# Nemo1999/Joint-TensoRF

Hardware: AMD Instinct MI355X
Metric: train rays/sec & Msamples/sec composited, lego VM-48, 1/2/4/8 MI355X (higher is better)
Workload: dtype f32; 1 GPU; bat_blender_VM stage 4: grid 400x400x400, S=1000 samples/ray, 1955 rays/iter/GPU (all_view_rand_grid lattice over 100 views), blur off, full train step (fwd+loss+bwd+Adam+pose Adam); samples_per_ray=1000, launch=eager, parallelism=1 GPU

## Files before the change

### joint_tensorf_amd/csrc/jt_shade.hip

```cpp
#include <atomic>
#include <cstdlib>

#include "jt_common.h"
#include "jt_walk.h"

#include "jt_shade_core.h"

#ifndef JT_B16_PINGPONG
#define JT_B16_PINGPONG 1
#endif
#ifndef JT_BF16X3_DEFAULT
#define JT_BF16X3_DEFAULT 7
#endif

namespace jt {

template <class C, int REC>
__global__ __launch_bounds__(256, 2) void k_shade_fwd(Dev D, MlpDev M, PeMask pm, const float* __restrict__ rays_o,
                                                      const float* __restrict__ rays_d,
                                                      const float* __restrict__ jitter,
                                                      const float* __restrict__ zvals,
                                                      const float* __restrict__ tmin,
                                                      const int* __restrict__ offset, int R,
                                                      const int* __restrict__ eray, const int* __restrict__ esmp,
                                                      const float* __restrict__ vdir, float* __restrict__ rgb_s,
                                                      float* __restrict__ rec, int cap, int rrows) {
  typedef BwdCfg<C> B;
  extern __shared__ __align__(16) float smem[];
  const int total = min(offset[R], cap);
  const int ntiles = (total + 31) >> 5;
  const int nblk = min((int)gridDim.x, (ntiles + 3) / 4);
  if ((int)blockIdx.x >= nblk) return;
  load_weights_lds<C>(smem, M);
  __syncthreads();
  const int lane = threadIdx.x & 63, wv = __builtin_amdgcn_readfirstlane(threadIdx.x >> 6);
  const int j_ = lane & 31, h_ = lane >> 5;
  constexpr int HOFF = (C::KIND == JT_MLP_FEA) ? 0 : 12;
  const XcdShare xs = xcd_share(ntiles, nblk);
  for (int tile = xs.lo + xs.rank * 4 + wv; tile < xs.hi; tile += xs.peers * 4) {
    int j = j_, h = h_;
    asm volatile("" : "+v"(j), "+v"(h));
    const int e = tile * 32 + j;
    const bool on = e < total;
    const int ee = on ? e : total - 1;
    float* rt = REC ? rec + (size_t)tile * (size_t)rrows * 32 : nullptr;
    EntryGeom g = entry_geom(D, rays_o, rays_d, jitter, zvals, tmin, eray, esmp, ee);
    float vd[3] = {vdir[(size_t)ee * 3], vdir[(size_t)ee * 3 + 1], vdir[(size_t)ee * 3 + 2]};
    if (REC && on && h == 0) {
#pragma unroll
      for (int c = 0; c < 3; ++c) {
        if (REC & 1) rec_st(rec_at(rt, B::R_VD + c, 4u * (unsigned)j), vd[c]);
        rec_st(rec_at(rt, B::R_GEO + c, 4u * (unsigned)j), g.n[c]);
      }
    }
    f32x16 facc = gather_basis<C, REC == 1>(D, smem, g.n, j, h, rt, on);
    if (REC) rec_store<1>(rt, B::R_F, &facc, j, h, on);
    Hidden<C> h1 = layer1<C>(smem, facc, vd, pm, j, h);
    relu_<C>(h1);
    if (REC) {
      unsigned mask1 = 0u;
#pragma unroll
      for (int mt = 0; mt < C::MT; ++mt)
#pragma unroll
        for (int r = 0; r < 16; ++r) mask1 |= (h1.v[mt][r] > 0.f) ? (1u << (mt * 16 + r)) : 0u;
      if (on) rec_st(rec_at(rt, B::R_MASK, 4u * (unsigned)j + 128u * (unsigned)h), __uint_as_float(mask1));
      if (REC & 1) rec_store<C::MT>(rt, B::R_H1, h1.v, j, h, on);
    }
    Hidden<C> h2 = layer2<C>(smem, h1, j, h);
    relu_<C>(h2);
    if (REC) {
      unsigned mask2 = 0u;
#pragma unroll
      for (int mt = 0; mt < C::MT; ++mt)
#pragma unroll
        for (int r = 0; r < 16; ++r) mask2 |= (h2.v[mt][r] > 0.f) ? (1u << (mt * 16 + r)) : 0u;
      if (on) rec_st(rec_at(rt, B::R_MASK + 2, 4u * (unsigned)j + 128u * (unsigned)h), __uint_as_float(mask2));
      if (REC & 1) rec_store<C::MT>(rt, B::R_MID + HOFF, h2.v, j, h, on);
      if ((REC & 1) && C::KIND != JT_MLP_FEA) {
        float pe[12];
        view_pe(vd, pm, pe);
        if (on && h == 0) {
#pragma unroll
          for (int k = 0; k < 12; ++k) rec_st(rec_at(rt, B::R_MID + k, 4u * (unsigned)j), pe[k]);
        }
      }
    }
    float o[3];
    layer3<C>(smem, h2, vd, pm, h, o);
    if (on && h == 0) {
#pragma unroll
      for (int c = 0; c < 3; ++c) rgb_s[(size_t)e * 3 + c] = 1.f / (1.f + expf(-o[c]));
    }
  }
}


#if JT_STAMP
__device__ unsigned long long g_stamps[8];
#define JT_STAMP_T() (__builtin_readcyclecounter())
#endif

template <class C, int REC>
__global__ __launch_bounds__(JT_B16_THREADS) void k_shade_fwd_b16(Dev D, MlpDev M, PeMask pm, const float* __restrict__ rays_o,
                                                      const float* __restrict__ rays_d,
                                                      const float* __restrict__ jitter,
                                                      const float* __restrict__ zvals,
                                                      const float* __restrict__ tmin,
                                                      const int* __restrict__ offset, int R,
                                                      const int* __restrict__ eray, const int* __restrict__ esmp,
                                                      const float* __restrict__ vdir, float* __restrict__ rgb_s,
                                                      float* __restrict__ rec, int cap, int rrows) {
  typedef BwdCfg<C> B;
  extern __shared__ __align__(16) unsigned char smem_raw[];
  typedef B16Cfg<C> Q;
  const uint4* img = reinterpret_cast<const uint4*>(smem_raw);
  const float* tail = reinterpret_cast<const float*>(smem_raw + (size_t)Q::V_END * 16);
  const float* smem = tail - C::O_W3;
  const int total = min(offset[R], cap);
  const int ntiles = (total + 31) >> 5;
  constexpr int NW = JT_B16_THREADS / 64;
  const int nblk = min((int)gridDim.x, (ntiles + NW - 1) / NW);
  if ((int)blockIdx.x >= nblk) return;
  load_weights_lds_b16<C>(smem_raw, M);
  __syncthreads();
  const int lane = threadIdx.x & 63, wv = __builtin_amdgcn_readfirstlane(threadIdx.x >> 6);
  const int j_ = lane & 31, h_ = lane >> 5;
  constexpr int HOFF = (C::KIND == JT_MLP_FEA) ? 0 : 12;
  const XcdShare xs = xcd_share(ntiles, nblk);
#if JT_SETPRIO
  if (wv >= NW / 2) __builtin_amdgcn_s_setprio(1);
#endif
  const int stride = xs.peers * NW;
  const int first = xs.lo + xs.rank * NW;
  const int iters0 = first < xs.hi ? (xs.hi - first + stride - 1) / stride : 0;
  f32x16 facc;
  float vd0 = 0.f, vd1 = 0.f, vd2 = 0.f;
  int e = 0;
  bool on = false, have = false;
  float* rt = nullptr;
#pragma unroll
  for (int r = 0; r < 16; ++r) facc[r] = 0.f;
#define JT_FWD_GATHER_STEP \
  {                                                                                                                    \
    int j = j_, h = h_; \
    asm volatile("" : "+v"(j), "+v"(h)); \
    e = tile * 32 + j; \
    on = e < total; \
    const int ee = on ? e : total - 1; \
    rt = REC ? rec + (size_t)tile * (size_t)rrows * 32 : nullptr; \
    EntryGeom g = entry_geom(D, rays_o, rays_d, jitter, zvals, tmin, eray, esmp, ee); \
    vd0 = vdir[(size_t)ee * 3], vd1 = vdir[(size_t)ee * 3 + 1], vd2 = vdir[(size_t)ee * 3 + 2]; \
    const float vd[3] = {vd0, vd1, vd2}; \
    if (REC && on && h == 0) { \
_Pragma("unroll") \
// ... 1098 lines not shown
  __shared__ float s_red[4][16][64];
  const int lane = threadIdx.x & 63, wv = threadIdx.x >> 6;
  const int m = lane & 31, h = lane >> 5;
  const int total = min(offset[R], cap);
  const int n = min(total - chunk_start, chunk_cap);
  if (n <= 0) return;
  const int ntiles = (n + 31) >> 5;
  const int per = wgrad_tiles_per_wave(n, gridDim.x);
  if ((int)blockIdx.x >= wgrad_active_blocks(n, gridDim.x)) return;
  const int w = blockIdx.x * 4 + wv;
  const int t_begin = min(w * per, ntiles), t_end = min(t_begin + per, ntiles);
  f32x16 acc[MT][NT];
  float asum[MT];
#pragma unroll
  for (int a = 0; a < MT; ++a) {
    asum[a] = 0.f;
#pragma unroll
    for (int b = 0; b < NT; ++b)
#pragma unroll
      for (int r = 0; r < 16; ++r) acc[a][b][r] = 0.f;
  }
  const size_t tstride = (size_t)rec_rows * 32;
  auto loadA = [&](int t, float (*dst)[16]) {
#pragma unroll
    for (int a = 0; a < MT; ++a) {
      const int c = a * 32 + m;
      load_row_half(rec + (size_t)t * tstride + (size_t)(a_row0 + min(c, M - 1)) * 32, c < M, h, dst[a]);
    }
  };
  auto prepA = [&](float (*av)[16], int nl, B3 (*a3)[2]) {
#pragma unroll
    for (int a = 0; a < MT; ++a) {
      if (nl < 32) mask_tail(av[a], h, nl);
#pragma unroll
      for (int q = 0; q < 16; ++q) asum[a] += av[a][q];
      a3[a][0] = split8(av[a]);
      a3[a][1] = split8(av[a] + 8);
    }
  };
  float av[MT][16], an[MT][16];
  B3 a3[MT][2];
  float gw[MT][3], raw[XA ? 4 : 1][16], rawn[XA ? 4 : 1][16];
  if (XA) {
#pragma unroll
    for (int a = 0; a < MT; ++a)
#pragma unroll
      for (int c = 0; c < 3; ++c) gw[a][c] = (a * 32 + m < M) ? gs.w3[c * gs.in3 + gs.hoff + a * 32 + m] : 0.f;
  }
  if (XF == 0) {
    auto loadB = [&](int t, int b, float* dst) {
      const int c = b * 32 + m;
      load_row_half(rec + (size_t)t * tstride + (size_t)(b_row0 + min(c, N - 1)) * 32, c < N, h, dst);
    };
    float bv[16], bn[16];
    if (t_begin < t_end) {
      if (XA) g2_load_raw(rec + (size_t)t_begin * tstride, gs, m, h, raw);
      else loadA(t_begin, av);
      loadB(t_begin, 0, bv);
    }
    for (int t = t_begin; t < t_end; ++t) {
      const int nl = min(32, n - t * 32);
#pragma unroll
      for (int b = 0; b < NT; ++b) {
        if (b + 1 < NT) {
          loadB(t, b + 1, bn);
        } else {
          const int tn = min(t + 1, t_end - 1);
          if (XA) g2_load_raw(rec + (size_t)tn * tstride, gs, m, h, rawn);
          else loadA(tn, an);
          loadB(tn, 0, bn);
        }
        if (b == 0) {
          if (XA) {
#pragma unroll
            for (int c = 0; c < 4; ++c) pin16(raw[XA ? c : 0]);
            g2_derive<MT>(raw, gw, m, av);
          } else {
#pragma unroll
          for (int a = 0; a < MT; ++a) pin16(av[a]);
          }
          prepA(av, nl, a3);
        }
        pin16(bv);
        if (nl < 32) mask_tail(bv, h, nl);
        const B3 b0 = split8(bv), b1 = split8(bv + 8);
#pragma unroll
        for (int a = 0; a < MT; ++a) {
          acc[a][b] = mfma6(a3[a][0], b0, acc[a][b]);
          acc[a][b] = mfma6(a3[a][1], b1, acc[a][b]);
        }
#pragma unroll
        for (int q = 0; q < 16; ++q) bv[q] = bn[q];
      }
      if (XA) {
#pragma unroll
        for (int c = 0; c < 4; ++c)
#pragma unroll
          for (int q = 0; q < 16; ++q) raw[XA ? c : 0][q] = rawn[XA ? c : 0][q];
      } else {
#pragma unroll
      for (int a = 0; a < MT; ++a)
#pragma unroll
        for (int q = 0; q < 16; ++q) av[a][q] = an[a][q];
      }
    }
  } else {
    const bool feat = m < APP, view = (XF == 1) && !feat && (m < APP + 3);
    const int srow = feat ? f_row0 + m : vd_row0 + (view ? m - APP : 0);
    const float m0 = view ? pm.v0 : pm.f0, m1 = view ? pm.v1 : pm.f1;
    const bool live = feat || view;
    float x[16], xn[16];
    if (t_begin < t_end) {
      loadA(t_begin, av);
      load_row_half(rec + (size_t)t_begin * tstride + (size_t)srow * 32, live, h, x);
    }
    for (int t = t_begin; t < t_end; ++t) {
      const int nl = min(32, n - t * 32);
      {
        const int tn = min(t + 1, t_end - 1);
        loadA(tn, an);
        load_row_half(rec + (size_t)tn * tstride + (size_t)srow * 32, live, h, xn);
      }
      pin16(x);
#pragma unroll
      for (int a = 0; a < MT; ++a) pin16(av[a]);
      if (nl < 32) mask_tail(x, h, nl);
      prepA(av, nl, a3);
      float sn[16], cs[16];
#pragma unroll
      for (int q = 0; q < 16; ++q) sincos_grad(x[q], &sn[q], &cs[q]);
#pragma unroll
      for (int b = 0; b < NT; ++b) {
        float bv[16];
#pragma unroll
        for (int q = 0; q < 16; ++q) bv[q] = live ? pe_pick<XF>(b, x[q], sn[q], cs[q], m0, m1) : 0.f;
        const B3 b0 = split8(bv), b1 = split8(bv + 8);
#pragma unroll
        for (int a = 0; a < MT; ++a) {
          acc[a][b] = mfma6(a3[a][0], b0, acc[a][b]);
          acc[a][b] = mfma6(a3[a][1], b1, acc[a][b]);
        }
      }
#pragma unroll
      for (int q = 0; q < 16; ++q) x[q] = xn[q];
#pragma unroll
      for (int a = 0; a < MT; ++a)
#pragma unroll
        for (int q = 0; q < 16; ++q) av[a][q] = an[a][q];
    }
  }
  wgrad_epilogue<MT, NT>(acc, asum, s_red, slab, lane, wv, m, h);
}

template <int MT, int NT, int XF>
__device__ inline void wgrad_reduce_body(int xblock, const float* __restrict__ slabs, int blocks_per_chunk,
                                         size_t chunk_stride, int chunk_entries, int total, int M, int N, int APP,
                                         float* __restrict__ dW, int ldw, float* __restrict__ db) {
  const int nchunks = (total + chunk_entries - 1) / chunk_entries;
  constexpr int PER = MT * NT * 1024 + MT * 32;
  const int idx = xblock * blockDim.x + threadIdx.x;
  if (idx >= PER) return;
  float s0 = 0.f, s1 = 0.f, s2 = 0.f, s3 = 0.f;
  const int gy = gridDim.y;
  for (int c = 0; c < nchunks; ++c) {
    const int active = wgrad_active_blocks(min(total - c * chunk_entries, chunk_entries), blocks_per_chunk);
    const float* base = slabs + (size_t)c * chunk_stride + idx;
    int q = blockIdx.y;
    for (; q + 3 * gy < active; q += 4 * gy) {
      s0 += base[(size_t)q * PER];
      s1 += base[(size_t)(q + gy) * PER];
      s2 += base[(size_t)(q + 2 * gy) * PER];
      s3 += base[(size_t)(q + 3 * gy) * PER];
    }
    for (; q < active; q += gy) s0 += base[(size_t)q * PER];
  }
  const float sum = (s0 + s1) + (s2 + s3);
  if (sum == 0.f) return;
  if (idx < MT * NT * 1024) {
    const int tile = idx >> 10, r = (idx >> 6) & 15, lane = idx & 63;
    const int a = tile / NT, b = tile - a * NT, m = lane & 31, h = lane >> 5;
    const int i = a * 32 + rowmap(r, 0) + 4 * h;
    const int k = (XF == 0) ? b * 32 + m : l1_column<XF>(b, m, APP);
    if (i < M && k >= 0 && k < N) atomicAdd(dW + (size_t)i * ldw + k, sum);
  } else if (db) {
    const int i = idx - MT * NT * 1024;
    if (i < M) atomicAdd(db + i, sum);
  }
}

template <class C>
struct WgradDims {
  static constexpr int NT3 = (C::IN3 + 31) / 32, NT1 = 5, NTB = (C::NC + 31) / 32;
  static constexpr size_t P3 = 1 * NT3 * 1024 + 32, P2 = (size_t)C::MT * C::MT * 1024 + C::MT * 32,
                          P1 = (size_t)C::MT * NT1 * 1024 + C::MT * 32, PB = 1 * NTB * 1024 + 32;
};

struct MlpGrad {
  float *basis, *w1, *b1, *w2, *b2, *w3, *b3;
};

template <class C>
__global__ __launch_bounds__(256) void k_wgrad_reduce4(const float* __restrict__ slabs, int blocks_per_chunk,
                                                       size_t chunk_stride, int chunk_entries,
                                                       const int* __restrict__ offset, int R, int cap, MlpGrad GM) {
  typedef WgradDims<C> W;
  constexpr int NT3 = W::NT3, NT1 = W::NT1, NTB = W::NTB;
  constexpr int XF1 = (C::KIND == JT_MLP_FEA) ? 1 : 2;
  constexpr int B3 = (int)((W::P3 + 255) / 256), B2 = (int)((W::P2 + 255) / 256), B1 = (int)((W::P1 + 255) / 256);
  const int total = min(offset[R], cap);
  const float* s3 = slabs;
  const float* s2 = s3 + W::P3 * blocks_per_chunk;
  const float* s1 = s2 + W::P2 * blocks_per_chunk;
  const float* sb = s1 + W::P1 * blocks_per_chunk;
  const int x = blockIdx.x;
  if (x < B3)
    wgrad_reduce_body<1, NT3, 0>(x, s3, blocks_per_chunk, chunk_stride, chunk_entries, total, 3, C::IN3, C::APP,
                                 GM.w3, C::IN3, GM.b3);
  else if (x < B3 + B2)
    wgrad_reduce_body<C::MT, C::MT, 0>(x - B3, s2, blocks_per_chunk, chunk_stride, chunk_entries, total, C::HID, C::HID,
                                       C::APP, GM.w2, C::HID, GM.b2);
  else if (x < B3 + B2 + B1)
    wgrad_reduce_body<C::MT, NT1, XF1>(x - B3 - B2, s1, blocks_per_chunk, chunk_stride, chunk_entries, total, C::HID,
                                       C::IN1, C::APP, GM.w1, C::IN1, GM.b1);
  else
    wgrad_reduce_body<1, NTB, 0>(x - B3 - B2 - B1, sb, blocks_per_chunk, chunk_stride, chunk_entries, total, C::APP, C::NC,
                                 C::APP, GM.basis, C::NC, (float*)nullptr);
}

}

using namespace jt;

static std::atomic<int> g_matrix_mode{-1};
static int bf16x3_mode() {
  int m = g_matrix_mode.load(std::memory_order_relaxed);
  if (m < 0) {
    const char* e = getenv("JT_BF16X3");
    m = (e ? atoi(e) : JT_BF16X3_DEFAULT) & 7;
    g_matrix_mode.store(m, std::memory_order_relaxed);
  }
  return m;
}

typedef ShadeCfg<48, 27, 64, JT_MLP_FEA> CfgBlender;
typedef ShadeCfg<20, 20, 32, JT_MLP_WEAKVIEW> CfgLlff;

static int shade_kind(const JtScene* s) {
  if (!s) return -1;
  if (s->view_pe != 2 || s->fea_pe != 2) return -1;
  if (s->n_comp_app == 48 && s->app_dim == 27 && s->mlp_hidden == 64 && s->mlp_kind == JT_MLP_FEA) return 0;
  if (s->n_comp_app == 20 && s->app_dim == 20 && s->mlp_hidden == 32 && s->mlp_kind == JT_MLP_WEAKVIEW) return 1;
  return -1;
}

static int g_chunk_log2 = 0;
static int chunk_entries() {
  if (!g_chunk_log2) {
    const char* e = getenv("JT_SHADE_CHUNK_LOG2");
    int l = e ? atoi(e) : 22;
    if (l < 16 || l > 22) l = 22;
    g_chunk_log2 = l;
  }
  return 1 << g_chunk_log2;
}
#if JT_STAMP
extern "C" int jt_debug_read_stamps(unsigned long long* out8) {
  if (hipMemcpyFromSymbol(out8, HIP_SYMBOL(g_stamps), 8 * sizeof(unsigned long long)) != hipSuccess) return JT_ERR_ARG;
  unsigned long long z[8] = {0, 0, 0, 0, 0, 0, 0, 0};
  if (hipMemcpyToSymbol(HIP_SYMBOL(g_stamps), z, sizeof(z)) != hipSuccess) return JT_ERR_ARG;
  return JT_OK;
}
#endif
static std::atomic<int> g_bwd_split{-2};
static int scatter_wgs(bool gemms_beside, bool lean = false, bool w12 = false) {
  static const int v = [] { const char* e = getenv("JT_SCATTER_WGS"); const int n = e ? atoi(e) : 0; return n > 0 ? n : 0; }();
  return v ? std::min(v, chip().cus) : chip().wgs(gemms_beside ? ((lean && !w12) ? 224 : 192) : 256);
}
static int bwd_split_mode() {
  int m = g_bwd_split.load(std::memory_order_relaxed);
  if (m < -1) {
    const char* e = getenv("JT_BWD_SPLIT");
    m = e ? atoi(e) : -1;
    if (m != 0 && m != 1 && m != 8 && m != 16) m = -1;
    g_bwd_split.store(m, std::memory_order_relaxed);
  }
  return m;
}
#if JT_TILE_STAMP
extern "C" int jt_debug_read_tile_stamps(unsigned long long* out16) {
  if (hipMemcpyFromSymbol(out16, HIP_SYMBOL(g_tstamps), 16 * sizeof(unsigned long long)) != hipSuccess) return JT_ERR_ARG;
  unsigned long long z[16] = {};
  if (hipMemcpyToSymbol(HIP_SYMBOL(g_tstamps), z, sizeof(z)) != hipSuccess) return JT_ERR_ARG;
  return JT_OK;
}
#endif
static std::atomic<int> g_lean{-1};
static int lean_mode() {
  int m = g_lean.load(std::memory_order_relaxed);
  if (m < 0) {
    const char* e = getenv("JT_LEAN_TAPE");
    m = (e ? atoi(e) : 1) ? 1 : 0;
    g_lean.store(m, std::memory_order_relaxed);
  }
  return m;
}
template <class C>
// ... 83 lines not shown
                             3 * (size_t)kTileMaxTiles * sizeof(int), 3 * (size_t)kTileMaxTiles * sizeof(int),
                             3 * (size_t)kTileMaxTiles * sizeof(int), 64 * sizeof(int)};
    for (int i = 0; i < 7; ++i) out[9 + 2 * i] = (int64_t)(uintptr_t)ptrs[i], out[10 + 2 * i] = (int64_t)sizes[i];
  }
}
extern "C" int jt_shade_workspace_layout(const JtScene* scene, int n_entries_max, int64_t* out23) {
  const int kind = shade_kind(scene);
  if (kind < 0 || !out23) return JT_ERR_UNSUPPORTED;
  if (n_entries_max < 1 || n_entries_max > kMaxEntries) return JT_ERR_ARG;
  if (kind == 0) ws_layout<CfgBlender>(n_entries_max, out23);
  else ws_layout<CfgLlff>(n_entries_max, out23);
  return JT_OK;
}

extern "C" int jt_shade_record_layout(const JtScene* scene, int32_t* out) {
  const int kind = shade_kind(scene);
  if (kind < 0 || !out) return JT_ERR_UNSUPPORTED;
  if (kind == 0) {
    out[0] = rec_rows<CfgBlender>(); out[1] = BwdCfg<CfgBlender>::R_MASK; out[2] = CfgBlender::HID;
  } else {
    out[0] = rec_rows<CfgLlff>(); out[1] = BwdCfg<CfgLlff>::R_MASK; out[2] = CfgLlff::HID;
  }
  out[3] = 32;
  return JT_OK;
}

template <class C, int REC>
static int launch_shade_fwd_t(const Dev& D, const MlpDev& M, const PeMask& pm, const float* rays_o,
                              const float* rays_d, const float* jitter, const float* zvals, const float* tmin,
                              const int32_t* offset, int R, const int32_t* eray, const int32_t* esmp,
                              const float* vdir, float* rgb_s, float* rec, int cap, hipStream_t st) {
  long tiles = ((long)cap + 31) / 32;
  if (bf16x3_mode() & 1) {
    const size_t lds16 = B16Cfg<C>::LDS_BYTES;
    (void)hipFuncSetAttribute(reinterpret_cast<const void*>(k_shade_fwd_b16<C, REC>),
                              hipFuncAttributeMaxDynamicSharedMemorySize, (int)lds16);
    constexpr int NW = JT_B16_THREADS / 64;
    int blocks16 = (int)std::min<long>((tiles + NW - 1) / NW, chip().cus);
    hipLaunchKernelGGL((k_shade_fwd_b16<C, REC>), dim3(blocks16), dim3(JT_B16_THREADS), lds16, st, D, M, pm, rays_o, rays_d, jitter,
                       zvals, tmin, offset, R, eray, esmp, vdir, rgb_s, rec, cap, rec_rows<C>());
    JT_LAUNCH_CHECK();
    return JT_OK;
  }
  const size_t lds = C::LDS_FLOATS * sizeof(float);
  (void)hipFuncSetAttribute(reinterpret_cast<const void*>(k_shade_fwd<C, REC>),
                            hipFuncAttributeMaxDynamicSharedMemorySize, (int)lds);
  int blocks = (int)std::min<long>((tiles + 3) / 4, 512);
  hipLaunchKernelGGL((k_shade_fwd<C, REC>), dim3(blocks), dim3(256), lds, st, D, M, pm, rays_o, rays_d, jitter, zvals,
                     tmin, offset, R, eray, esmp, vdir, rgb_s, rec, cap, rec_rows<C>());
  JT_LAUNCH_CHECK();
  return JT_OK;
}

template <class C>
static int launch_shade_fwd(const Dev& D, const MlpDev& M, const PeMask& pm, const float* rays_o,
                            const float* rays_d, const float* jitter, const float* zvals, const float* tmin,
                            const int32_t* offset, int R, const int32_t* eray, const int32_t* esmp,
                            const float* vdir, float* rgb_s, int cap, float* ws, size_t ws_bytes, int flags,
                            hipStream_t st) {
  if (ws) {
    if (ws_bytes < WsLayout<C>::bytes(cap)) return JT_ERR_ARG;
    if (flags & JT_SHADE_POSE_ONLY)
      return launch_shade_fwd_t<C, 2>(D, M, pm, rays_o, rays_d, jitter, zvals, tmin, offset, R, eray, esmp, vdir,
                                      rgb_s, ws, cap, st);
    if (lean_tape<C>())
      return launch_shade_fwd_t<C, 3>(D, M, pm, rays_o, rays_d, jitter, zvals, tmin, offset, R, eray, esmp, vdir,
                                      rgb_s, ws, cap, st);
    return launch_shade_fwd_t<C, 1>(D, M, pm, rays_o, rays_d, jitter, zvals, tmin, offset, R, eray, esmp, vdir,
                                    rgb_s, ws, cap, st);
  }
  return launch_shade_fwd_t<C, 0>(D, M, pm, rays_o, rays_d, jitter, zvals, tmin, offset, R, eray, esmp, vdir,
                                  rgb_s, nullptr, cap, st);
}

extern "C" int jt_shade_forward(const JtScene* scene, const JtFactors* factors, const JtMlp* mlp, const float* rays_o,
                                const float* rays_d, const float* jitter, const float* zvals, const float* tmin,
                                const int32_t* shade_offset, int n_rays, const int32_t* entry_ray,
                                const int32_t* entry_smp, const float* viewdirs, float* rgb_s, int n_entries_max,
                                void* workspace, size_t workspace_bytes, int flags, void* stream) {
  Dev D;
  int rc = make_dev(scene, factors, &D);
  if (rc) return rc;
  if (!factors || !mlp || !rays_o || !rays_d || !tmin || !shade_offset || !entry_ray || !entry_smp || !viewdirs ||
      !rgb_s)
    return JT_ERR_ARG;
  if (!mlp->basis || !mlp->w1 || !mlp->b1 || !mlp->w2 || !mlp->b2 || !mlp->w3 || !mlp->b3) return JT_ERR_ARG;
  if (D.ndc && !zvals) return JT_ERR_ARG;
  const int kind = shade_kind(scene);
  if (kind < 0) return JT_ERR_UNSUPPORTED;
  if (n_entries_max < 1) return JT_OK;
  if (n_entries_max > kMaxEntries) return JT_ERR_ARG;
  MlpDev M = {mlp->basis, mlp->w1, mlp->b1, mlp->w2, mlp->b2, mlp->w3, mlp->b3};
  PeMask pm = pe_masks(scene->fea_pe_progress, scene->view_pe_progress, scene->fea_pe, scene->view_pe);
  hipStream_t st = (hipStream_t)stream;
  if (kind == 0)
    return launch_shade_fwd<CfgBlender>(D, M, pm, rays_o, rays_d, jitter, zvals, tmin, shade_offset, n_rays,
                                        entry_ray, entry_smp, viewdirs, rgb_s, n_entries_max, (float*)workspace,
                                        workspace_bytes, flags, st);
  return launch_shade_fwd<CfgLlff>(D, M, pm, rays_o, rays_d, jitter, zvals, tmin, shade_offset, n_rays, entry_ray,
                                   entry_smp, viewdirs, rgb_s, n_entries_max, (float*)workspace, workspace_bytes, flags,
                                   st);
}

template <class C>
struct TileSel {
  static constexpr int NG = (C::CA + 15) / 16;
  static constexpr int SPLIT0 = (NG >= 3) ? 2 : 0;
  static int ch_max(int cfg) { return (cfg == 0 && SPLIT0) ? 16 * SPLIT0 : C::CA; }
  static int waves(int cfg) { return cfg == 0 ? 16 : 8; }
  static size_t lds_bytes(int cfg, int line_len) { return tile_lds_bytes(line_len, ch_max(cfg), waves(cfg)); }
  static int tiles(int H, int W) { return tiles_along(W) * tiles_along(H); }
  template <int CFG>
  static int launch(const Dev& D, const MlpDev& M, const JtFactors& G, const TileWs& TW, const int32_t* offset, int R,
                    float* g_xyz, const float* rc, int start, int ccap, int cap, int line_len, hipStream_t st) {
    constexpr int SPLIT = CFG == 0 ? SPLIT0 : 0;
    constexpr int WAVES = CFG == 0 ? 16 : 8;
    constexpr int NCLS = SPLIT ? 2 : 1;
    int nt[3], ntmax = 1;
    for (int a = 0; a < 3; ++a) nt[a] = tiles(D.ph[a], D.pw[a]), ntmax = std::max(ntmax, nt[a]);
    const int nblk = (ccap + 255) / 256;
    hipLaunchKernelGGL(k_tile_zero, dim3((ntmax + 255) / 256, 3), dim3(256), 0, st, TW, nt[0], nt[1], nt[2]);
    hipLaunchKernelGGL((k_tile_bin<C, false>), dim3(nblk), dim3(256), 0, st, D, TW, offset, R, rc, start, ccap, cap);
    hipLaunchKernelGGL(k_tile_scan, dim3(3), dim3(1024), 0, st, TW, nt[0], nt[1], nt[2]);
    hipLaunchKernelGGL((k_tile_bin<C, true>), dim3(nblk), dim3(256), 0, st, D, TW, offset, R, rc, start, ccap, cap);
    const size_t lds = lds_bytes(CFG, line_len);
    static size_t attr = 0;
    if (attr < lds) {
      if (hipFuncSetAttribute(reinterpret_cast<const void*>(k_tile_scatter<C, SPLIT, WAVES>),
                              hipFuncAttributeMaxDynamicSharedMemorySize, (int)lds) != hipSuccess)
        return JT_ERR_UNSUPPORTED;
      attr = lds;
    }
    static const int nwg_env = [] { const char* e = getenv("JT_TILE_WGS"); const int v = e ? atoi(e) : 0; return v >= 6 ? v : 0; }();
    const int nwg = nwg_env ? nwg_env : std::max(chip().cus, 6);
    static const int ratio = [] { const char* e = getenv("JT_TILE_RATIO"); const int v = e ? atoi(e) : 0; return (v > 0 && v < 100) ? v : 62; }();
    TileClasses TC;
    int acc = 0;
    for (int pl = 0; pl < 3; ++pl) {
      const int share = nwg / 3 + (pl < nwg % 3 ? 1 : 0);
      const int c0 = NCLS == 2 ? std::max(1, std::min(share - 1, share * ratio / 100)) : share;
      TC.start[pl * NCLS] = acc;
      acc += c0;
      if (NCLS == 2) {
        TC.start[pl * NCLS + 1] = acc;
        acc += share - c0;
      }
    }
    for (int k = 3 * NCLS; k <= kTileMaxClasses; ++k) TC.start[k] = acc;
    hipLaunchKernelGGL((k_tile_scatter<C, SPLIT, WAVES>), dim3(acc), dim3(WAVES * 64), lds, st, D, M, G, TW, rc, TC);
    hipLaunchKernelGGL(k_tile_gxyz, dim3(nblk), dim3(256), 0, st, TW, 3 * NCLS, offset, R, g_xyz, start, ccap, cap);
    return JT_OK;
  }
};

template <class C>
static int launch_shade_bwd(const Dev& D, const MlpDev& M, const PeMask& pm, const JtFactors& G, const JtMlp& GM,
                            const int32_t* offset, int R, const float* rgb_s, const float* g_rgb_s, float* g_xyz,
                            int cap,
                            float* ws, size_t ws_bytes, int flags, hipStream_t st, hipStream_t aux,
                            hipEvent_t ev_fork, hipEvent_t ev_join) {
  typedef BwdCfg<C> B;
  typedef WsLayout<C> W;
  const size_t lds = B::LDS_FLOATS * sizeof(float);
  if (lds > 160 * 1024) return JT_ERR_UNSUPPORTED;
  if (ws_bytes < W::bytes(cap)) return JT_ERR_ARG;
  const int chunk = kChunkEntries;
  const int nchunks = (int)(((long)cap + chunk - 1) / chunk);
  (void)hipFuncSetAttribute(reinterpret_cast<const void*>(k_shade_bwd<C, false>),
                            hipFuncAttributeMaxDynamicSharedMemorySize, (int)lds);
  (void)hipFuncSetAttribute(reinterpret_cast<const void*>(k_shade_bwd<C, true>),
                            hipFuncAttributeMaxDynamicSharedMemorySize, (int)lds);
  float* recs = ws;
  float* slabs = ws + W::rec_floats(cap);
  const size_t cstride = W::slab_floats_per_chunk();
  const int nb = kWgradBlocks;
  static const int abl_env = [] { const char* e = getenv("JT_ABLATE"); return e ? atoi(e) : 0; }();
  const int det = jt_deterministic();
  const int ablate = abl_env | ((flags & JT_SHADE_SKIP_WGRAD) ? 4 : 0) |
                     ((flags & kNoGradRecords) ? 2 : 0) | (det ? 16 : 0) | (lean_tape<C>() ? 32 : 0);
  constexpr int NT3 = W::NT3, NT1 = W::NT1, NTB = W::NTB;
  constexpr int XF1 = (C::KIND == JT_MLP_FEA) ? 1 : 2;
  const bool use_aux = aux && ev_fork && ev_join && !(ablate & 4);
  static const bool pipe = [] { const char* e = getenv("JT_WGRAD_PIPE"); return !e || atoi(e) != 0; }();
  hipStream_t ws_st = use_aux ? aux : st;
  const int RR = rec_rows<C>();
  const int split_dflt = split_default<C>();
  int split = bwd_split_mode() >= 0 ? bwd_split_mode() : split_dflt;
  unsigned* bad = jt::fixed_bad_flag();
  if (!bad) return JT_ERR_ARG;
  typedef TileSel<C> TS;
  int tile_line_len = 0;
  for (int a = 0; a < 3; ++a) tile_line_len = std::max(tile_line_len, D.ll[a]);
  const int tile_cfg = 1;
  if (split == 1) {
    bool ok = !det && G.app_plane[0] && G.app_line[0] && TS::lds_bytes(tile_cfg, tile_line_len) <= 160 * 1024;
    for (int a = 0; a < 3 && ok; ++a) ok = TS::tiles(D.ph[a], D.pw[a]) <= kTileMaxTiles;
    if (!ok) split = split_dflt;
  }
  const bool tile = (split == 1);
  const TileWs TW = tile_ws_carve(reinterpret_cast<char*>(ws) + W::main_bytes(cap), cap, chunk);
  static const bool pose_env = [] { const char* e = getenv("JT_POSE_BWD"); return !e || atoi(e) != 0; }();
  const bool pose_only = pose_env && !det && !G.app_plane[0] && !G.app_line[0] && (flags & kNoGradRecords) && (ablate & 4);
  if (pose_only) split = 16;
  const bool lean = lean_tape<C>();
  if (lean && (split != 8 && split != 16)) return JT_ERR_ARG;
  const bool dbs = lean && !pose_only && !(ablate & 4) && GM.basis != nullptr;
  if (dbs && (size_t)chip().cus * ScatCfg<C>::DB_SLAB > W::PB * (size_t)kWgradBlocks) return JT_ERR_UNSUPPORTED;
  auto launch_bwd = [&](int ci) -> int {
    const int start = ci * chunk, ccap = std::min(chunk, cap - start);
    long tiles = ((long)ccap + 31) / 32;
    int blocks = (int)std::min<long>((tiles + B::NWAVE - 1) / B::NWAVE, chip().cus);
    float* rc = recs + W::rec_floats_per_chunk() * ci;
    if (split && (bf16x3_mode() & 4)) {
      const size_t lds_b = ((BwdB16Cfg<C>::IMG_BYTES + 15) & ~(size_t)15) + (size_t)B::NWAVE * B::STASH_FLOATS * sizeof(float);
      static bool attr_b = false;
      if (!attr_b) {
        (void)hipFuncSetAttribute(reinterpret_cast<const void*>(k_shade_bwd<C, false, true, true>),
                                  hipFuncAttributeMaxDynamicSharedMemorySize, (int)lds_b);
        attr_b = true;
      }
      hipLaunchKernelGGL((k_shade_bwd<C, false, true, true>), dim3(blocks), dim3(512), lds_b, st, D, M, pm, G, offset, R, rgb_s,
                         g_rgb_s, g_xyz, rc, start, ccap, cap, ablate, bad, RR);
    } else if (split) {
      const size_t lds_c = B::LDS_FLOATS_SPLIT * sizeof(float);
      static bool attr_done = false;
      if (!attr_done) {
        (void)hipFuncSetAttribute(reinterpret_cast<const void*>(k_shade_bwd<C, false, true>),
                                  hipFuncAttributeMaxDynamicSharedMemorySize, (int)lds_c);
        attr_done = true;
      }
      hipLaunchKernelGGL((k_shade_bwd<C, false, true>), dim3(blocks), dim3(512), lds_c, st, D, M, pm, G, offset, R, rgb_s,
                         g_rgb_s, g_xyz, rc, start, ccap, cap, ablate, bad, RR);
    } else if (det) {
      hipLaunchKernelGGL((k_shade_bwd<C, true>), dim3(blocks), dim3(512), lds, st, D, M, pm, G, offset, R, rgb_s,
                         g_rgb_s, g_xyz, rc, start, ccap, cap, ablate, bad, RR);
    } else {
      hipLaunchKernelGGL((k_shade_bwd<C, false>), dim3(blocks), dim3(512), lds, st, D, M, pm, G, offset, R, rgb_s,
                         g_rgb_s, g_xyz, rc, start, ccap, cap, ablate, bad, RR);
    }
    JT_LAUNCH_CHECK();
    return JT_OK;
  };
  static const int sflags_env = [] { const char* e = getenv("JT_SCATTER_FLAGS"); return e ? atoi(e) & 1 : 1; }();
  int line_floats = 0;
  for (int a = 0; a < 3; ++a) line_floats = std::max(line_floats, D.ll[a] * C::CA);
  int sflags = split ? sflags_env : 0;
  if (det) sflags &= ~1;
  auto scatter_lds = [&](int run, int fl, int sw) {
    return (size_t)(ScatCfg<C>::BT_FLOATS + ((fl & 1) ? line_floats : 0) + (dbs ? ScatCfg<C>::RED_FLOATS : 0) +
                    sw * ScatCfg<C>::wave_floats(run, dbs)) * sizeof(float);
  };
  static const int sw_env = [] { const char* e = getenv("JT_SCATTER_WAVES"); return e ? atoi(e) : 0; }();
  int sw = 8;
  if (C::CA < 48 && split && !tile && (sw_env == 16 || (sw_env == 0 && scatter_lds(split, sflags, 16) <= 160 * 1024))) sw = 16;
  bool w12 = false;
  if (C::CA >= 48 && !det && !tile && !pose_only && dbs && sflags == 1 && (sw_env == 0 || sw_env == 12) &&
      ((bwd_split_mode() == -1 && split == 16) || (bwd_split_mode() == 8 && sw_env == 12)) &&
      scatter_lds(8, sflags, 12) <= 160 * 1024) {
    split = 8, sw = 12, w12 = true;
  }
  if (split && !tile && scatter_lds(split, sflags, sw) > 160 * 1024) sflags &= ~1;
  auto launch_scatter = [&](int ci) -> int {
    if (!split || (ablate & 1)) return JT_OK;
    const int start = ci * chunk, ccap = std::min(chunk, cap - start);
    const float* rc = recs + W::rec_floats_per_chunk() * ci;
    if (pose_only) {
      const long tiles = ((long)ccap + 31) / 32;
      const int pblocks = (int)std::min<long>((tiles + 3) / 4, 2048L);
      if ((bf16x3_mode() & 4) && C::CA >= 48)
        hipLaunchKernelGGL((k_pose_gather<C, (C::CA >= 48)>), dim3(pblocks), dim3(256), 0, st, D, M, offset, R, g_xyz, rc, start, ccap, cap, RR);
      else
        hipLaunchKernelGGL((k_pose_gather<C, false>), dim3(pblocks), dim3(256), 0, st, D, M, offset, R, g_xyz, rc, start, ccap, cap, RR);
      JT_LAUNCH_CHECK();
      return JT_OK;
    }
    if (tile) {
      int rc_ = TS::template launch<1>(D, M, G, TW, offset, R, g_xyz, rc, start, ccap, cap, tile_line_len, st);
      if (rc_) return rc_;
      JT_LAUNCH_CHECK();
      return JT_OK;
    }
    const size_t lds_s = scatter_lds(split, sflags, sw);
#define JT_SCATTER_LAUNCH(RUN_, DET_, FL_, SW_)                                                                         \
  {                                                                                                                     \
    static bool attr = false;                                                                                           \
    if (!attr) {                                                                                                        \
      (void)hipFuncSetAttribute(reinterpret_cast<const void*>(k_shade_scatter<C, DET_, RUN_, SW_, FL_>),                \
                                hipFuncAttributeMaxDynamicSharedMemorySize, 160 * 1024);                                \
      attr = true;                                                                                                      \
    }                                                                                                                   \
    const long nbatch = ((long)ccap + 4 * RUN_ - 1) / (4 * RUN_);                                                       \
    const int sblocks = (int)std::min<long>((nbatch + SW_ - 1) / SW_, (long)scatter_wgs(use_aux && C::CA >= 48, dbs, w12));                             \
    hipLaunchKernelGGL((k_shade_scatter<C, DET_, RUN_, SW_, FL_>), dim3(sblocks), dim3(SW_ * 64), lds_s, st, D, M, G,   \
                       offset, R, g_xyz, rc, start, ccap, cap, bad, line_floats, RR,                                    \
                       slabs + (size_t)ci * cstride + (W::P3 + W::P2 + W::P1) * nb);                                    \
  }
#define JT_SCATTER_FL(RUN_, SW_)                                                                \
  {                                                                                             \
    if (det && dbs) JT_SCATTER_LAUNCH(RUN_, true, 2, SW_)                                       \
    else if (det) JT_SCATTER_LAUNCH(RUN_, true, 0, SW_)                                         \
    else if (sflags == 1 && dbs) JT_SCATTER_LAUNCH(RUN_, false, 3, SW_)                         \
    else if (sflags == 1) JT_SCATTER_LAUNCH(RUN_, false, 1, SW_)                                \
    else if (dbs) JT_SCATTER_LAUNCH(RUN_, false, 2, SW_)                                        \
    else JT_SCATTER_LAUNCH(RUN_, false, 0, SW_)                                                 \
  }
#define JT_SCATTER_RUN(RUN_)                                                                    \
  {                                                                                             \
    if (C::CA < 48 && sw == 16) JT_SCATTER_FL(RUN_, (C::CA < 48 ? 16 : 8))                      \
    else JT_SCATTER_FL(RUN_, 8)                                                                 \
  }
    if (w12)
      JT_SCATTER_LAUNCH(8, false, 3, (C::CA >= 48 ? 12 : 8))
    else if (split == 8) JT_SCATTER_RUN(8) else JT_SCATTER_RUN(16)
#undef JT_SCATTER_RUN
#undef JT_SCATTER_FL
#undef JT_SCATTER_LAUNCH
    JT_LAUNCH_CHECK();
    return JT_OK;
  };
  auto launch_wgrad = [&](int ci) -> int {
    const int start = ci * chunk, ccap = std::min(chunk, cap - start);
    const float* rec = recs + W::rec_floats_per_chunk() * ci;
    const G2Src gs = {M.w3, B::R_GO, B::R_MASK + 2, C::IN3, (C::KIND == JT_MLP_FEA) ? 0 : 12};
    float* s3 = slabs + (size_t)ci * cstride;
    float* s2 = s3 + W::P3 * nb;
    float* s1 = s2 + W::P2 * nb;
    float* sb = s1 + W::P1 * nb;
#define JT_WGRAD_LAUNCH(KERNEL)                                                                                          \
  hipLaunchKernelGGL((KERNEL<1, NT3, 0>), dim3(nb), dim3(256), 0, ws_st, rec, B::R_GO, 3, B::R_MID, C::IN3, B::R_F,      \
                     B::R_VD, RR, pm, C::APP, offset, R, cap, start, ccap, s3, gs);                                      \
  JT_LAUNCH_CHECK();                                                                                                     \
  if (lean) {                                                                                                            \
  hipLaunchKernelGGL((KERNEL<C::MT, C::MT, 0, 1>), dim3(nb), dim3(256), 0, ws_st, rec, B::R_G2, C::HID, B::R_H1, C::HID, \
                     B::R_F, B::R_VD, RR, pm, C::APP, offset, R, cap, start, ccap, s2, gs);                              \
  } else {                                                                                                               \
  hipLaunchKernelGGL((KERNEL<C::MT, C::MT, 0>), dim3(nb), dim3(256), 0, ws_st, rec, B::R_G2, C::HID, B::R_H1, C::HID,    \
                     B::R_F, B::R_VD, RR, pm, C::APP, offset, R, cap, start, ccap, s2, gs);                              \
  }                                                                                                                      \
  JT_LAUNCH_CHECK();                                                                                                     \
  hipLaunchKernelGGL((KERNEL<C::MT, NT1, XF1>), dim3(nb), dim3(256), 0, ws_st, rec, B::R_G1, C::HID, B::R_F, C::IN1,     \
                     B::R_F, B::R_VD, RR, pm, C::APP, offset, R, cap, start, ccap, s1, gs);                              \
  JT_LAUNCH_CHECK();                                                                                                     \
  if (!dbs) {                                                                                                            \
  hipLaunchKernelGGL((KERNEL<1, NTB, 0>), dim3(nb), dim3(256), 0, ws_st, rec, B::R_GF, C::APP, B::R_PROD, C::NC, B::R_F, \
                     B::R_VD, RR, pm, C::APP, offset, R, cap, start, ccap, sb, gs);                                      \
  JT_LAUNCH_CHECK();                                                                                                     \
  }
    if (bf16x3_mode() & 2) {
      JT_WGRAD_LAUNCH(k_wgrad_b16)
    } else {
      JT_WGRAD_LAUNCH(k_wgrad)
    }
#undef JT_WGRAD_LAUNCH
    return JT_OK;
  };
  static const bool scatter_first = [] { const char* e = getenv("JT_SCATTER_FIRST"); return e && atoi(e) != 0; }();
  for (int ci = 0; ci < nchunks; ++ci) {
    int rc = launch_bwd(ci);
    if (rc) return rc;
    if (scatter_first && (rc = launch_scatter(ci))) return rc;
    if (use_aux && pipe) {
      if (hipEventRecord(ev_fork, st) != hipSuccess) return JT_ERR_ARG;
      if (hipStreamWaitEvent(aux, ev_fork, 0) != hipSuccess) return JT_ERR_ARG;
      if ((rc = launch_wgrad(ci))) return rc;
    }
    if (!scatter_first && (rc = launch_scatter(ci))) return rc;
  }
  if (dbs && !(ablate & 1)) {
    const int ry = det ? 1 : 8;
    hipLaunchKernelGGL((k_dbasis_reduce<C>), dim3((ScatCfg<C>::DB_SLAB + 255) / 256, ry), dim3(256), 0, st,
                       slabs + (W::P3 + W::P2 + W::P1) * nb, cstride, chunk, scatter_wgs(use_aux && C::CA >= 48, dbs, w12), 4 * split,
                       sw, offset, R, cap, GM.basis);
    JT_LAUNCH_CHECK();
  }
  if (ablate & 4) return JT_OK;
  if (use_aux && !pipe) {
    if (hipEventRecord(ev_fork, st) != hipSuccess) return JT_ERR_ARG;
    if (hipStreamWaitEvent(aux, ev_fork, 0) != hipSuccess) return JT_ERR_ARG;
  }
  if (!use_aux && ev_fork && hipEventRecord(ev_fork, st) != hipSuccess) return JT_ERR_ARG;
  if (!(use_aux && pipe)) {
    for (int ci = 0; ci < nchunks; ++ci) {
      int rc = launch_wgrad(ci);
      if (rc) return rc;
    }
  }
  {
    const int ry = det ? 1 : 32;
    const int nblk = (int)((W::P3 + 255) / 256 + (W::P2 + 255) / 256 + (W::P1 + 255) / 256 + (dbs ? 0 : (W::PB + 255) / 256));
    const MlpGrad gm = {GM.basis, GM.w1, GM.b1, GM.w2, GM.b2, GM.w3, GM.b3};
    hipLaunchKernelGGL((k_wgrad_reduce4<C>), dim3(nblk, ry), dim3(256), 0, ws_st, slabs, nb, cstride, chunk, offset, R, cap,
                       gm);
    JT_LAUNCH_CHECK();
  }
  if (ws_st != st) {
    if (hipEventRecord(ev_join, aux) != hipSuccess) return JT_ERR_ARG;
  }
  return JT_OK;
}

extern "C" int jt_shade_backward(const JtScene* scene, const JtFactors* factors, const JtMlp* mlp,
                                 const float* rays_o, const float* rays_d, const float* jitter, const float* zvals,
                                 const float* tmin, const int32_t* shade_offset, int n_rays,
                                 const int32_t* entry_ray, const int32_t* entry_smp, const float* viewdirs,
                                 const float* rgb_s, const float* g_rgb_s, const JtFactors* g_factors, const JtMlp* g_mlp,
                                 float* g_xyz_app, int n_entries_max, void* workspace, size_t workspace_bytes,
                                 int flags, void* stream, void* aux_stream, void* ev_fork, void* ev_join) {
  Dev D;
  int rc = make_dev(scene, factors, &D);
  if (rc) return rc;
  if (!factors || !mlp || !rays_o || !rays_d || !tmin || !shade_offset || !entry_ray ||
      !entry_smp || !viewdirs || !rgb_s || !g_rgb_s || !g_xyz_app)
    return JT_ERR_ARG;
  if (!mlp->basis || !mlp->w1 || !mlp->b1 || !mlp->w2 || !mlp->b2 || !mlp->w3 || !mlp->b3) return JT_ERR_ARG;
  if (g_mlp && (!g_mlp->basis || !g_mlp->w1 || !g_mlp->b1 || !g_mlp->w2 || !g_mlp->b2 || !g_mlp->w3 || !g_mlp->b3))
    return JT_ERR_ARG;
  for (int a = 0; a < 3; ++a)
    if (g_factors && (!g_factors->app_plane[a] || !g_factors->app_line[a])) return JT_ERR_ARG;
  JtFactors no_fac = {};
  JtMlp no_mlp = {};
  if (!g_mlp) flags |= JT_SHADE_SKIP_WGRAD | kNoGradRecords;
  const JtFactors& GFr = g_factors ? *g_factors : no_fac;
  const JtMlp& GMr = g_mlp ? *g_mlp : no_mlp;
  if (D.ndc && !zvals) return JT_ERR_ARG;
  const int kind = shade_kind(scene);
  if (kind < 0) return JT_ERR_UNSUPPORTED;
  if (n_entries_max < 1) return JT_OK;
  if (!workspace || n_entries_max > kMaxEntries) return JT_ERR_ARG;
  MlpDev M = {mlp->basis, mlp->w1, mlp->b1, mlp->w2, mlp->b2, mlp->w3, mlp->b3};
  PeMask pm = pe_masks(scene->fea_pe_progress, scene->view_pe_progress, scene->fea_pe, scene->view_pe);
  hipStream_t st = (hipStream_t)stream;
  if (kind == 0)
    return launch_shade_bwd<CfgBlender>(D, M, pm, GFr, GMr, shade_offset, n_rays, rgb_s, g_rgb_s, g_xyz_app,
                                        n_entries_max, (float*)workspace, workspace_bytes, flags, st, (hipStream_t)aux_stream,
                                        (hipEvent_t)ev_fork, (hipEvent_t)ev_join);
  return launch_shade_bwd<CfgLlff>(D, M, pm, GFr, GMr, shade_offset, n_rays, rgb_s, g_rgb_s, g_xyz_app,
                                   n_entries_max,
                                   (float*)workspace, workspace_bytes, flags, st, (hipStream_t)aux_stream,
                                   (hipEvent_t)ev_fork, (hipEvent_t)ev_join);
}
```

Measured before the change: 728,800 rays/s.

## Add fused weight-gradient kernel and move dbasis reduce to aux stream

Adds an opt-in kernel that computes the layer-3, layer-2 and layer-1 weight-gradient partial slabs in one pass over each record tile, replacing three separate launches and re-reads of the records. Separately, when the aux pipeline is active, the dbasis reduction is moved from the main stream to the aux stream behind an event, so the main stream can continue while it runs. The fused path has more register pressure and runs only when an environment variable is set. The stream move adds a per-device cached event and changes the order of work on the aux stream.

```diff
diff --git a/joint_tensorf_amd/csrc/jt_shade.hip b/joint_tensorf_amd/csrc/jt_shade.hip
--- a/joint_tensorf_amd/csrc/jt_shade.hip
+++ b/joint_tensorf_amd/csrc/jt_shade.hip
@@ -1,5 +1,6 @@
 #include <atomic>
 #include <cstdlib>
+#include <mutex>
 
 #include "jt_common.h"
 #include "jt_walk.h"
@@ -1404,6 +1405,177 @@
   wgrad_epilogue<MT, NT>(acc, asum, s_red, slab, lane, wv, m, h);
 }
 
+struct WgradRows {
+  int mid, h1, g1, f, vd, rec_rows;
+};
+
+template <int MTA>
+__device__ inline void wgrad_prep_a(float (*av)[16], int nl, int h, float* asum, B3 (*a3)[2]) {
+#pragma unroll
+  for (int a = 0; a < MTA; ++a) {
+    if (nl < 32) mask_tail(av[a], h, nl);
+#pragma unroll
+    for (int q = 0; q < 16; ++q) asum[a] += av[a][q];
+    a3[a][0] = split8(av[a]);
+    a3[a][1] = split8(av[a] + 8);
+  }
+}
+
+template <int MT, int NT3, int XF>
+__global__ __launch_bounds__(256) void k_wgrad_fused(const float* __restrict__ rec, WgradRows RW, int IN3, PeMask pm, int APP,
+                                                     const int* __restrict__ offset, int R, int cap, int chunk_start,
+                                                     int chunk_cap, float* __restrict__ slab3, float* __restrict__ slab2,
+                                                     float* __restrict__ slab1, G2Src gs) {
+  constexpr int HID = MT * 32, NT1 = 5;
+  __shared__ float s_red[4][16][64];
+  const int lane = threadIdx.x & 63, wv = threadIdx.x >> 6;
+  const int m = lane & 31, h = lane >> 5;
+  const int total = min(offset[R], cap);
+  const int n = min(total - chunk_start, chunk_cap);
+  if (n <= 0) return;
+  const int ntiles = (n + 31) >> 5;
+  const int per = wgrad_tiles_per_wave(n, gridDim.x);
+  if ((int)blockIdx.x >= wgrad_active_blocks(n, gridDim.x)) return;
+  const int w = blockIdx.x * 4 + wv;
+  const int t_begin = min(w * per, ntiles), t_end = min(t_begin + per, ntiles);
+  f32x16 acc3[1][NT3], acc2[MT][MT], acc1[MT][NT1];
+  float asum3[1] = {0.f}, asum2[MT], asum1[MT];
+#pragma unroll
+  for (int r = 0; r < 16; ++r) {
+#pragma unroll
+    for (int b = 0; b < NT3; ++b) acc3[0][b][r] = 0.f;
+#pragma unroll
+    for (int a = 0; a < MT; ++a) {
+#pragma unroll
+      for (int b = 0; b < MT; ++b) acc2[a][b][r] = 0.f;
+#pragma unroll
+      for (int b = 0; b < NT1; ++b) acc1[a][b][r] = 0.f;
+    }
+  }
+#pragma unroll
+  for (int a = 0; a < MT; ++a) asum2[a] = asum1[a] = 0.f;
+  const size_t tstride = (size_t)RW.rec_rows * 32;
+  auto loadRow = [&](int t, int row0, int c, int N, float* dst) {
+    load_row_half(rec + (size_t)t * tstride + (size_t)(row0 + min(c, N - 1)) * 32, true, h, dst);
+  };
+  auto zero_dead = [&](float* v, bool alive) {
+#pragma unroll
+    for (int q = 0; q < 16; ++q) v[q] = alive ? v[q] : 0.f;
+  };
+  float gw[MT][3];
+#pragma unroll
+  for (int a = 0; a < MT; ++a)
+#pragma unroll
+    for (int c = 0; c < 3; ++c) gw[a][c] = gs.w3[c * gs.in3 + gs.hoff + a * 32 + m];
+  const bool feat = m < APP, view = (XF == 1) && !feat && (m < APP + 3);
+  const int srow = feat ? RW.f + m : RW.vd + (view ? m - APP : 0);
+  const float m0 = view ? pm.v0 : pm.f0, m1 = view ? pm.v1 : pm.f1;
+  const bool live = feat || view;
+  const unsigned k0 = (m == 0) ? ~0u : 0u, k1 = (m == 1) ? ~0u : 0u, k2 = (m == 2) ? ~0u : 0u;
+  float raw[4][16], bv[16];
+  if (t_begin < t_end) {
+    g2_load_raw(rec + (size_t)t_begin * tstride, gs, m, h, raw);
+    loadRow(t_begin, RW.mid, m, IN3, bv);
+  }
+  for (int t = t_begin; t < t_end; ++t) {
+    const int nl = min(32, n - t * 32);
+    {
+      B3 a3[1][2];
+#pragma unroll
+      for (int b = 0; b < NT3; ++b) {
+        float bn[16];
+        if (b + 1 < NT3) loadRow(t, RW.mid, (b + 1) * 32 + m, IN3, bn);
+        else loadRow(t, RW.h1, m, HID, bn);
+        if (b == 0) {
+#pragma unroll
+          for (int c = 0; c < 4; ++c) pin16(raw[c]);
+          float av[1][16];
+#pragma unroll
+          for (int q = 0; q < 16; ++q)
+            av[0][q] = __uint_as_float((__float_as_uint(raw[0][q]) & k0) | (__float_as_uint(raw[1][q]) & k1) |
+                                       (__float_as_uint(raw[2][q]) & k2));
+          wgrad_prep_a<1>(av, nl, h, asum3, a3);
+        }
+        pin16(bv);
+        if ((b + 1) * 32 > IN3) zero_dead(bv, b * 32 + m < IN3);
+        if (nl < 32) mask_tail(bv, h, nl);
+        const B3 b0 = split8(bv), b1 = split8(bv + 8);
+        acc3[0][b] = mfma6(a3[0][0], b0, acc3[0][b]);
+        acc3[0][b] = mfma6(a3[0][1], b1, acc3[0][b]);
+#pragma unroll
+        for (int q = 0; q < 16; ++q) bv[q] = bn[q];
+      }
+    }
+    float an[MT][16], xn[16];
+    {
+      B3 a3[MT][2];
+#pragma unroll
+      for (int b = 0; b < MT; ++b) {
+        float bn[16];
+        if (b + 1 < MT) {
+          loadRow(t, RW.h1, (b + 1) * 32 + m, HID, bn);
+        } else {
+#pragma unroll
+          for (int a = 0; a < MT; ++a) loadRow(t, RW.g1, a * 32 + m, HID, an[a]);
+          load_row_half(rec + (size_t)t * tstride + (size_t)srow * 32, true, h, xn);
+        }
+        if (b == 0) {
+          float av[MT][16];
+          g2_derive<MT>(raw, gw, m, av);
+          wgrad_prep_a<MT>(av, nl, h, asum2, a3);
+        }
+        pin16(bv);
+        if (nl < 32) mask_tail(bv, h, nl);
+        const B3 b0 = split8(bv), b1 = split8(bv + 8);
+#pragma unroll
+        for (int a = 0; a < MT; ++a) {
+          acc2[a][b] = mfma6(a3[a][0], b0, acc2[a][b]);
+          acc2[a][b] = mfma6(a3[a][1], b1, acc2[a][b]);
+        }
+        if (b + 1 < MT) {
+#pragma unroll
+          for (int q = 0; q < 16; ++q) bv[q] = bn[q];
+        }
+      }
+    }
+    {
+      const int tn = min(t + 1, t_end - 1);
+      const float* tile_n = rec + (size_t)tn * tstride;
+#pragma unroll
+      for (int c = 0; c < 3; ++c) load_row_half(tile_n + (size_t)(gs.go_row0 + c) * 32, true, h, raw[c]);
+      pin16(xn);
+#pragma unroll
+      for (int a = 0; a < MT; ++a) pin16(an[a]);
+      zero_dead(xn, live);
+      if (nl < 32) mask_tail(xn, h, nl);
+      B3 a3[MT][2];
+      wgrad_prep_a<MT>(an, nl, h, asum1, a3);
+      float sn[16], cs[16];
+#pragma unroll
+      for (int q = 0; q < 16; ++q) sincos_grad(xn[q], &sn[q], &cs[q]);
+      constexpr int order[NT1] = {0, 3, 2, 1, 4};
+#pragma unroll
+      for (int i = 0; i < NT1; ++i) {
+        const int b = order[i];
+        float xb[16];
+#pragma unroll
+        for (int q = 0; q < 16; ++q) xb[q] = live ? pe_pick<XF>(b, xn[q], sn[q], cs[q], m0, m1) : 0.f;
+        const B3 b0 = split8(xb), b1 = split8(xb + 8);
+        if (i == 0) loadRow(tn, RW.mid, m, IN3, bv);
+        if (i == 2) load_row_half(tile_n + (size_t)(gs.mask_row0 + ((m >> 2) & 1)) * 32, true, h, raw[3]);
+#pragma unroll
+        for (int a = 0; a < MT; ++a) {
+          acc1[a][b] = mfma6(a3[a][0], b0, acc1[a][b]);
+          acc1[a][b] = mfma6(a3[a][1], b1, acc1[a][b]);
+        }
+      }
+    }
+  }
+  wgrad_epilogue<1, NT3>(acc3, asum3, s_red, slab3, lane, wv, m, h);
+  wgrad_epilogue<MT, MT>(acc2, asum2, s_red, slab2, lane, wv, m, h);
+  wgrad_epilogue<MT, NT1>(acc1, asum1, s_red, slab1, lane, wv, m, h);
+}
+
 template <int MT, int NT, int XF>
 __device__ inline void wgrad_reduce_body(int xblock, const float* __restrict__ slabs, int blocks_per_chunk,
                                          size_t chunk_stride, int chunk_entries, int total, int M, int N, int APP,
@@ -1793,6 +1965,24 @@
     return JT_OK;
   }
 };
+
+static hipEvent_t dbasis_event() {
+  static hipEvent_t ev[64] = {};
+  static std::atomic<int> state[64] = {};
+  int dev = 0;
+  if (hipGetDevice(&dev) != hipSuccess || dev < 0 || dev >= 64) return nullptr;
+  int s = state[dev].load(std::memory_order_acquire);
+  if (s == 0) {
+    static std::mutex mu;
+    std::lock_guard<std::mutex> lock(mu);
+    if (state[dev].load(std::memory_order_acquire) == 0) {
+      const bool ok = hipEventCreateWithFlags(&ev[dev], hipEventDisableTiming) == hipSuccess;
+      state[dev].store(ok ? 1 : 2, std::memory_order_release);
+    }
+    s = state[dev].load(std::memory_order_acquire);
+  }
+  return s == 1 ? ev[dev] : nullptr;
+}
 
 template <class C>
 static int launch_shade_bwd(const Dev& D, const MlpDev& M, const PeMask& pm, const JtFactors& G, const JtMlp& GM,
@@ -1959,6 +2149,8 @@
     JT_LAUNCH_CHECK();
     return JT_OK;
   };
+  static const bool fused_env = [] { const char* e = getenv("JT_WGRAD_FUSED"); return e && atoi(e) != 0; }();
+  const bool wgrad_fused = fused_env && (bf16x3_mode() & 2) && lean && dbs;
   auto launch_wgrad = [&](int ci) -> int {
     const int start = ci * chunk, ccap = std::min(chunk, cap - start);
     const float* rec = recs + W::rec_floats_per_chunk() * ci;
@@ -1987,7 +2179,12 @@
                      B::R_VD, RR, pm, C::APP, offset, R, cap, start, ccap, sb, gs);                                      \
   JT_LAUNCH_CHECK();                                                                                                     \
   }
-    if (bf16x3_mode() & 2) {
+    if (wgrad_fused) {
+      const WgradRows rw = {B::R_MID, B::R_H1, B::R_G1, B::R_F, B::R_VD, RR};
+      hipLaunchKernelGGL((k_wgrad_fused<C::MT, NT3, XF1>), dim3(nb), dim3(256), 0, ws_st, rec, rw, C::IN3, pm, C::APP, offset, R,
+                         cap, start, ccap, s3, s2, s1, gs);
+      JT_LAUNCH_CHECK();
+    } else if (bf16x3_mode() & 2) {
       JT_WGRAD_LAUNCH(k_wgrad_b16)
     } else {
       JT_WGRAD_LAUNCH(k_wgrad)
@@ -2007,12 +2204,20 @@
     }
     if (!scatter_first && (rc = launch_scatter(ci))) return rc;
   }
-  if (dbs && !(ablate & 1)) {
+  const bool dbr_aux = dbs && !(ablate & 1) && use_aux && pipe && dbasis_event() != nullptr;
+  auto launch_dbasis_reduce = [&](hipStream_t s) {
     const int ry = det ? 1 : 8;
-    hipLaunchKernelGGL((k_dbasis_reduce<C>), dim3((ScatCfg<C>::DB_SLAB + 255) / 256, ry), dim3(256), 0, st,
+    hipLaunchKernelGGL((k_dbasis_reduce<C>), dim3((ScatCfg<C>::DB_SLAB + 255) / 256, ry), dim3(256), 0, s,
                        slabs + (W::P3 + W::P2 + W::P1) * nb, cstride, chunk, scatter_wgs(use_aux && C::CA >= 48, dbs, w12), 4 * split,
                        sw, offset, R, cap, GM.basis);
-    JT_LAUNCH_CHECK();
+  };
+  if (dbs && !(ablate & 1)) {
+    if (dbr_aux) {
+      if (hipEventRecord(dbasis_event(), st) != hipSuccess) return JT_ERR_ARG;
+    } else {
+      launch_dbasis_reduce(st);
+      JT_LAUNCH_CHECK();
+    }
   }
   if (ablate & 4) return JT_OK;
   if (use_aux && !pipe) {
@@ -2032,6 +2237,11 @@
     const MlpGrad gm = {GM.basis, GM.w1, GM.b1, GM.w2, GM.b2, GM.w3, GM.b3};
     hipLaunchKernelGGL((k_wgrad_reduce4<C>), dim3(nblk, ry), dim3(256), 0, ws_st, slabs, nb, cstride, chunk, offset, R, cap,
                        gm);
+    JT_LAUNCH_CHECK();
+  }
+  if (dbr_aux) {
+    if (hipStreamWaitEvent(aux, dbasis_event(), 0) != hipSuccess) return JT_ERR_ARG;
+    launch_dbasis_reduce(aux);
     JT_LAUNCH_CHECK();
   }
   if (ws_st != st) {
```

Result: no change. 728,700 rays/s (-0.0%).
